# autonomousvision/LaRa

Hardware: AMD Instinct MI355X
Metric: novel-view frames/sec @512x512 (4-view in, 2DGS fwd+bwd) (higher is better)
Workload: dtype f32 raster + bf16-MFMA/f32-accumulate encoder (+ bf16-autocast coarse decoder MLP, as the reference's bf16-mixed)

## Files before the change

lara_amd/coarse.py:

```python
from __future__ import annotations

import torch
from torch import nn

from ._native import call, query, require_device

_F, _FA, _O = 80, 88, 48


class _CoarseDecoder(torch.autograd.Function):
    @staticmethod
    def forward(ctx, x, w1, b1, w2, b2, w3, b3, K, sh_dim, opacity_shift, scaling_shift):
        require_device(x)
        f = lambda t: t.detach().float().contiguous()
        x, w1, b1, w2, b2, w3, b3 = map(f, (x, w1, b1, w2, b2, w3, b3))
        M, n_par = x.shape[0], K * (10 + sh_dim)
        if (x.shape != (M, _F) or w1.shape != (_F, _F) or w2.shape != (_F, _F) or w3.shape != (n_par, _F) or n_par > _O
                or b1.shape != (_F,) or b2.shape != (_F,) or b3.shape != (n_par,)):
            raise RuntimeError("expected x [M,80], Linear(80,80), Linear(80,80), Linear(80, K*(10+sh_dim) <= 48)")
        new = lambda c: torch.empty(M, K * c, dtype=torch.float32, device=x.device)
        offset, sh, scaling, rotation, opacity = new(3), new(sh_dim), new(2), new(4), new(1)
        call("lara_coarse_decoder_forward", x.device, M, K, sh_dim, x, w1, b1, w2, b2, w3, b3, float(opacity_shift),
             float(scaling_shift), offset, sh, scaling, rotation, opacity)
        ctx.save_for_backward(x, w1, b1, w2, b2, w3, offset)
        ctx.dims = (M, K, sh_dim, n_par)
        ctx.set_materialize_grads(False)
        return offset, sh, scaling, rotation, opacity

    @staticmethod
    def backward(ctx, g_offset, g_sh, g_scaling, g_rotation, g_opacity):
        x, w1, b1, w2, b2, w3, offset = ctx.saved_tensors
        M, K, sh_dim, n_par = ctx.dims
        gs = [None if g is None else g.float().contiguous() for g in (g_offset, g_sh, g_scaling, g_rotation, g_opacity)]
        dev = x.device
        Mp = query("lara_coarse_decoder_padded_rows", M)
        dx = torch.empty_like(x)
        cols = (_FA, _FA, _FA, _F, _F, _O)
        slab = torch.empty(Mp * sum(cols), dtype=torch.bfloat16, device=dev)
        mats, o = [], 0
        for c in cols:
            mats.append(slab[o:o + Mp * c].view(Mp, c))
            o += Mp * c
        xb, h1, h2, dz1, dz2, dz3 = mats
        grads = torch.zeros((2 * _F + _O) * _FA, dtype=torch.float32, device=dev)
        g1, g2, g3 = grads[:_F * _FA].view(_F, _FA), grads[_F * _FA:2 * _F * _FA].view(_F, _FA), grads[2 * _F * _FA:].view(_O, _FA)
        ws = torch.empty(query("lara_gemm_tn_workspace_bytes"), dtype=torch.uint8, device=dev)
        call("lara_coarse_decoder_backward", dev, M, K, sh_dim, x, w1, b1, w2, b2, w3, offset, *gs, dx, xb, h1, h2, dz1, dz2, dz3)
        if M:
            for dz, act, g in ((dz1, xb, g1), (dz2, h1, g2), (dz3, h2, g3)):
                call("lara_gemm_tn_bf16", dev, Mp, dz.shape[1], _FA, dz, act, g, ws)
        return (dx, g1[:, :_F], g1[:, _F], g2[:, :_F], g2[:, _F], g3[:n_par, :_F], g3[:n_par, _F], None, None, None, None)


def supported(decoder) -> bool:
    seq = getattr(decoder, "mlp_coarse", None)
    if any(not hasattr(decoder, a) for a in ("K", "sh_dim", "opacity_dim", "scaling_dim", "rotation_dim")):
        return False
    if seq is None or len(seq) != 5 or not all(isinstance(seq[i], nn.Linear) for i in (0, 2, 4)):
        return False
    if not all(isinstance(seq[i], nn.ReLU) for i in (1, 3)) or any(seq[i].bias is None for i in (0, 2, 4)):
        return False
    return (tuple(seq[0].weight.shape) == (_F, _F) and tuple(seq[2].weight.shape) == (_F, _F)
            and tuple(seq[4].weight.shape) == (decoder.K * (10 + decoder.sh_dim), _F) and seq[4].weight.shape[0] <= _O
            and decoder.opacity_dim == 1 and decoder.scaling_dim == 2 and decoder.rotation_dim == 4)


def forward_coarse(decoder, feats, opacity_shift, scaling_shift):
    if not supported(decoder):
        raise RuntimeError("lara_amd.coarse: mlp_coarse must be Linear(80,80) ReLU Linear(80,80) ReLU Linear(80, K*(10+sh_dim) <= 48)")
    seq, K, B = decoder.mlp_coarse, decoder.K, feats.shape[0]
    offset, sh, scaling, rotation, opacity = _CoarseDecoder.apply(
        feats.reshape(-1, feats.shape[-1]), seq[0].weight, seq[0].bias, seq[2].weight, seq[2].bias, seq[4].weight, seq[4].bias,
        K, decoder.sh_dim, opacity_shift, scaling_shift)
    return (offset.view(B, -1, 3), sh.view(B, -1, decoder.sh_dim // 3, 3), scaling.view(B, -1, 2), rotation.view(B, -1, 4),
            opacity.view(B, -1, 1))
```

lara_amd/csrc/coarsedec.hip:

```cpp
#include "common.h"
#include "../../include/lara_coarsedec.h"

namespace {

typedef __attribute__((ext_vector_type(4))) short s16x4;
typedef __attribute__((ext_vector_type(4))) float f32x4;

__device__ __forceinline__ unsigned short f2bf(const float f) {
    unsigned u = __float_as_uint(f);
    u += 0x7fffu + ((u >> 16) & 1u);
    return (unsigned short)(u >> 16);
}
__device__ __forceinline__ float bf2f(const unsigned short h) { return __uint_as_float((unsigned)h << 16); }

constexpr int CD_F = 80;
constexpr int CD_O = 48;
constexpr int CD_LDW = 84;
constexpr int CD_PTS = 128;
constexpr int CD_NB = 208;
constexpr int CD_FA = 88;
constexpr int CD_TILE = 16 * CD_O + 16 * 12;
constexpr int CD_WG_FWD = 1024, CD_WG_BWD = 512;

struct CdP {
    int M, n_par;
    const float *x, *w1, *b1, *w2, *b2, *w3, *b3;
    float *out[5];
    const float *dout[5];
    const float *offset_out;
    float *dx;
    unsigned short *xb, *h1, *h2, *dz1, *dz2, *dz3;
    float opacity_shift, scaling_shift;
    int width[5], toff[5];
    signed char tensor[CD_O], col[CD_O], act[CD_O];
};

template <int ROWS>
__device__ __forceinline__ void stage_matrix(const float *__restrict__ w, const int rows_valid, unsigned short *dst,
                                             const int ld, const bool transposed) {
    constexpr int N = ROWS * CD_F, TRIPS = (N + 255) / 256;
    float v[TRIPS];
#pragma unroll
    for (int u = 0; u < TRIPS; u++) {
        const int idx = u * 256 + (int)threadIdx.x;
        v[u] = (idx < N && idx < rows_valid * CD_F) ? w[idx] : 0.f;
    }
#pragma unroll
    for (int u = 0; u < TRIPS; u++) {
        const int idx = u * 256 + (int)threadIdx.x;
        if (idx >= N) continue;
        const int r = idx / CD_F, c = idx - r * CD_F;
        if (transposed) dst[c * ld + r] = f2bf(v[u]); else dst[r * ld + c] = f2bf(v[u]);
    }
}
__device__ __forceinline__ void stage_bias(const float *__restrict__ b, const int n_valid, const int n, float *dst) {
    for (int i = threadIdx.x; i < n; i += 256) dst[i] = i < n_valid ? bf2f(f2bf(b[i])) : 0.f;
}

typedef __attribute__((ext_vector_type(4))) __bf16 bf16x4;
template <int NI, int NT, bool TR>
__device__ __forceinline__ void mm(const unsigned short *Ws, const int ld, const float *bs, const s16x4 (&in)[NT][2],
                                   f32x4 (&acc)[NI][2], const int c16, const int q4) {
#pragma unroll
    for (int i = 0; i < NI; i++) {
        f32x4 b = {0.f, 0.f, 0.f, 0.f};
        if (bs) b = *(const f32x4 *)(bs + 16 * i + 4 * q4);
        acc[i][0] = b; acc[i][1] = b;
#pragma unroll
        for (int t = 0; t < NT; t++) {
            s16x4 a;
            if (TR) {
                const unsigned short *src = Ws + (16 * t + 4 * q4 + (c16 >> 2)) * ld + 16 * i + 4 * (c16 & 3);
                a = __builtin_bit_cast(s16x4, __builtin_amdgcn_ds_read_tr16_b64_v4bf16((__attribute__((address_space(3))) bf16x4 *)src));
            } else {
                a = *(const s16x4 *)(Ws + (16 * i + c16) * ld + 16 * t + 4 * q4);
            }
            acc[i][0] = __builtin_amdgcn_mfma_f32_16x16x16bf16_1k(a, in[t][0], acc[i][0], 0, 0, 0);
            acc[i][1] = __builtin_amdgcn_mfma_f32_16x16x16bf16_1k(a, in[t][1], acc[i][1], 0, 0, 0);
        }
    }
}

__device__ __forceinline__ s16x4 pack4(const float a, const float b, const float c, const float d) {
// ... 198 lines not shown
            const float *tl = tile + c * CD_TILE;
#pragma unroll
            for (int i = 0; i < 3; i++) {
                float v[4];
#pragma unroll
                for (int r = 0; r < 4; r++) {
                    v[r] = 0.f;
                    if (slot[i][r] < 0) continue;
                    float g = tl[slot[i][r]];
                    if ((is_offset >> (4 * i + r)) & 1u) {
                        const float o = tl[16 * CD_O + slot[i][r]];
                        g *= 0.5f * (1.0f - o * o);
                    }
                    v[r] = g;
                }
                g3[i][c] = pack4(v[0], v[1], v[2], v[3]);
            }
        }
        __builtin_amdgcn_wave_barrier();
        asm volatile("s_waitcnt lgkmcnt(0)" ::: "memory");
        store_frags<3, false>(p.dz3, CD_O, base, c16, q4, g3);
        mm<5, 3, true>(W3s, CD_LDW, nullptr, g3, acc, c16, q4);
#pragma unroll
        for (int i = 0; i < 5; i++)
#pragma unroll
            for (int c = 0; c < 2; c++) {
                const bool in_range = base + 16 * c + c16 < p.M;
#pragma unroll
                for (int e = 0; e < 4; e++) {
                    const unsigned short h = (in_range && ((live2[c] >> (4 * i + e)) & 1u)) ? f2bf(acc[i][c][e]) : (unsigned short)0;
                    a[i][c][e] = (short)h;
                }
            }
        store_frags<5, false>(p.dz2, CD_F, base, c16, q4, a);
        mm<5, 5, true>(W2s, CD_LDW, nullptr, a, acc, c16, q4);
#pragma unroll
        for (int i = 0; i < 5; i++)
#pragma unroll
            for (int c = 0; c < 2; c++) {
                const bool in_range = base + 16 * c + c16 < p.M;
#pragma unroll
                for (int e = 0; e < 4; e++) {
                    const unsigned short h = (in_range && ((live1[c] >> (4 * i + e)) & 1u)) ? f2bf(acc[i][c][e]) : (unsigned short)0;
                    b[i][c][e] = (short)h;
                }
            }
        store_frags<5, false>(p.dz1, CD_F, base, c16, q4, b);
        mm<5, 5, true>(W1s, CD_LDW, nullptr, b, acc, c16, q4);
#pragma unroll
        for (int c = 0; c < 2; c++) {
            const int row = base + 16 * c + c16;
            if (row >= p.M) continue;
            float4 *dst = (float4 *)(p.dx + (size_t)row * CD_F) + q4;
#pragma unroll
            for (int i = 0; i < 5; i++) dst[4 * i] = make_float4(acc[i][c][0], acc[i][c][1], acc[i][c][2], acc[i][c][3]);
        }
    }
}

int fill_map(CdP &p, const int K, const int sh_dim) {
    const int per = 10 + sh_dim;
    if (K < 1 || sh_dim < 0 || K * per > CD_O) return LARA2DGS_E_INVALID;
    static_assert(CD_TILE - 16 * CD_O >= 16 * 3 * (CD_O / 10), "the backward's copy of `offset` (16 x 3K floats) must fit the tile's tail for every K with 10 K <= CD_O");
    p.n_par = K * per;
    const int widths[5] = {3, sh_dim, 2, 4, 1};
    for (int t = 0, o = 0; t < 5; t++) { p.width[t] = K * widths[t]; p.toff[t] = o; o += 16 * p.width[t]; }
    for (int q = 0; q < CD_O; q++) { p.tensor[q] = 0; p.col[q] = 0; p.act[q] = 0; }
    for (int k = 0; k < K; k++)
        for (int j = 0; j < per; j++) {
            int t, c, a = 0;
            if (j < 3) { t = 0; c = j; a = 1; }
            else if (j < 3 + sh_dim) { t = 1; c = j - 3; }
            else if (j < 4 + sh_dim) { t = 4; c = 0; a = 3; }
            else if (j < 6 + sh_dim) { t = 2; c = j - 4 - sh_dim; a = 2; }
            else { t = 3; c = j - 6 - sh_dim; }
            const int q = k * per + j;
            p.tensor[q] = (signed char)t; p.col[q] = (signed char)(k * widths[t] + c); p.act[q] = (signed char)a;
        }
    return LARA2DGS_OK;
}

}

extern "C" {

int64_t lara_coarse_decoder_padded_rows(int64_t M) { return (M + CD_PTS - 1) / CD_PTS * CD_PTS; }

int lara_coarse_decoder_forward(int32_t M, int32_t K, int32_t sh_dim, const float *x, const float *w1, const float *b1,
                                const float *w2, const float *b2, const float *w3, const float *b3, float opacity_shift,
                                float scaling_shift, float *offset, float *sh, float *scaling, float *rotation,
                                float *opacity, void *stream) {
    if (M < 0 || !w1 || !b1 || !w2 || !b2 || !w3 || !b3) return LARA2DGS_E_INVALID;
    CdP p{};
    if (int rc = fill_map(p, K, sh_dim)) return rc;
    if (M == 0) return LARA2DGS_OK;
    if (!x || !offset || !scaling || !rotation || !opacity || (sh_dim > 0 && !sh)) return LARA2DGS_E_INVALID;
    p.M = M; p.x = x; p.w1 = w1; p.b1 = b1; p.w2 = w2; p.b2 = b2; p.w3 = w3; p.b3 = b3;
    p.out[0] = offset; p.out[1] = sh; p.out[2] = scaling; p.out[3] = rotation; p.out[4] = opacity;
    p.opacity_shift = opacity_shift; p.scaling_shift = scaling_shift;
    const int trips = (M + CD_PTS - 1) / CD_PTS;
    L2D_LAUNCH("coarse_decoder_fwd", (hipStream_t)stream, coarse_fwd_kernel, dim3(trips < CD_WG_FWD ? trips : CD_WG_FWD), dim3(256), 0, p);
    return LARA2DGS_OK;
}

int lara_coarse_decoder_backward(int32_t M, int32_t K, int32_t sh_dim, const float *x, const float *w1, const float *b1,
                                 const float *w2, const float *b2, const float *w3, const float *offset_out,
                                 const float *d_offset, const float *d_sh, const float *d_scaling, const float *d_rotation,
                                 const float *d_opacity, float *dx, uint16_t *xb, uint16_t *h1, uint16_t *h2,
                                 uint16_t *dz1, uint16_t *dz2, uint16_t *dz3, void *stream) {
    if (M < 0 || !w1 || !b1 || !w2 || !b2 || !w3) return LARA2DGS_E_INVALID;
    CdP p{};
    if (int rc = fill_map(p, K, sh_dim)) return rc;
    hipStream_t s = (hipStream_t)stream;
    if (M == 0) return LARA2DGS_OK;
    if (!x || !dx || !xb || !h1 || !h2 || !dz1 || !dz2 || !dz3 || (d_offset && !offset_out)) return LARA2DGS_E_INVALID;
    p.M = M; p.x = x; p.w1 = w1; p.b1 = b1; p.w2 = w2; p.b2 = b2; p.w3 = w3;
    p.dout[0] = d_offset; p.dout[1] = d_sh; p.dout[2] = d_scaling; p.dout[3] = d_rotation; p.dout[4] = d_opacity;
    p.offset_out = offset_out; p.dx = dx;
    p.xb = xb; p.h1 = h1; p.h2 = h2; p.dz1 = dz1; p.dz2 = dz2; p.dz3 = dz3;
    const int trips = (M + CD_PTS - 1) / CD_PTS;
    const int grid = trips < CD_WG_BWD ? trips : CD_WG_BWD;
    L2D_LAUNCH("coarse_decoder_bwd", s, coarse_bwd_kernel, dim3(grid), dim3(256), 0, p);
    return LARA2DGS_OK;
}

}
```

lara_amd/csrc/pointfeat.hip:

```cpp
#include "common.h"
#include "../../include/lara_pointfeat.h"

namespace {

constexpr int PF_MAX_VIEWS = 8;

struct PfP {
    int n, V, h, w;
    const float *points, *w2cs, *ixts, *img_ref, *image, *acc, *depth;
    int vtot;
};

__device__ __forceinline__ size_t map_pixel(const PfP &p, const size_t i) {
    if (p.vtot == 0) return i;
    const size_t hw = (size_t)p.h * p.w, v = i / hw, pix = i - v * hw, y = pix / p.w, x = pix - y * p.w;
    return (y * p.vtot + v) * p.w + x;
}

struct Tap {
    int idx[4];
    float wgt[4];
    float wx, wy;
    bool in[4];
};

__device__ __forceinline__ Tap taps(const float x, const float y, const int h, const int w) {
    Tap t;
    const float fx = floorf(x), fy = floorf(y);
    t.wx = x - fx; t.wy = y - fy;
    const int x0 = (fx >= -2.f && fx <= (float)w + 1.f) ? (int)fx : -2, y0 = (fy >= -2.f && fy <= (float)h + 1.f) ? (int)fy : -2;
#pragma unroll
    for (int k = 0; k < 4; k++) {
        const int xi = x0 + (k & 1), yi = y0 + (k >> 1);
        t.in[k] = xi >= 0 && xi < w && yi >= 0 && yi < h;
        t.idx[k] = t.in[k] ? yi * w + xi : 0;
        t.wgt[k] = ((k & 1) ? t.wx : 1.f - t.wx) * ((k >> 1) ? t.wy : 1.f - t.wy);
    }
    return t;
}

__global__ void __launch_bounds__(256)
pack_stack_kernel(const PfP p, float4 *__restrict__ packed) {
    const size_t hw = (size_t)p.h * p.w, i = (size_t)blockIdx.x * 256 + threadIdx.x;
    if (i >= (size_t)p.V * hw) return;
    const size_t v = i / hw, pix = i - v * hw, m = map_pixel(p, i);
    const float *im = p.image + m * 3;
    packed[2 * i] = make_float4(p.img_ref[(v * 3 + 0) * hw + pix], p.img_ref[(v * 3 + 1) * hw + pix],
                                p.img_ref[(v * 3 + 2) * hw + pix], im[0]);
    packed[2 * i + 1] = make_float4(im[1], im[2], p.acc[m], p.depth[m]);
}

__global__ void __launch_bounds__(256)
unpack_grad_kernel(const PfP p, const float4 *__restrict__ dpacked, const size_t n, float *d_image, float *d_acc, float *d_depth) {
    const size_t i = (size_t)blockIdx.x * 256 + threadIdx.x;
// ... 138 lines not shown
    L2D_LAUNCH_IN_SCOPE(s, (point_feats_bwd_kernel<VP>), dim3((unsigned)((threads + 255) / 256)), dim3(256), 0, p, packed, g_out,
                        d_points, dpacked);
    return LARA2DGS_OK;
}
int launch_pack(const PfP &p, float4 *packed, hipStream_t s) {
    const size_t n = (size_t)p.V * p.h * p.w;
    L2D_LAUNCH_IN_SCOPE(s, pack_stack_kernel, dim3((unsigned)((n + 255) / 256)), dim3(256), 0, p, packed);
    return LARA2DGS_OK;
}

struct RowsP {
    const float *src[LARA_ROWS_MAX];
    float *dst[LARA_ROWS_MAX];
    int width[LARA_ROWS_MAX], first[LARA_ROWS_MAX + 1];
    const int64_t *idx;
    int n, count;
};
template <bool SCATTER>
__global__ void __launch_bounds__(256) take_rows_kernel(const RowsP p) {
    const int total = p.first[p.count];
    const int t = blockIdx.x * 256 + threadIdx.x;
    if (t >= p.n * total) return;
    const int r = t / total, c = t - r * total;
    int k = 0;
    while (k + 1 < p.count && c >= p.first[k + 1]) k++;
    const int w = p.width[k], cc = c - p.first[k];
    const size_t far = (size_t)p.idx[r] * w + cc, near = (size_t)r * w + cc;
    if (SCATTER) p.dst[k][far] = p.src[k][near];
    else p.dst[k][near] = p.src[k][far];
}

__global__ void __launch_bounds__(256) voxel_rows_fwd_kernel(const int n, const int c4, const long long *__restrict__ vox,
                                                            const float4 *__restrict__ x, float4 *__restrict__ out) {
    const long long t = (long long)blockIdx.x * 256 + threadIdx.x;
    if (t >= (long long)n * c4) return;
    const int r = (int)(t / c4), c = (int)(t - (long long)r * c4);
    out[t] = x[(size_t)vox[r] * c4 + c];
}
__global__ void __launch_bounds__(256) voxel_rows_bwd_kernel(const int n, const int c4, const long long *__restrict__ vox,
                                                            const float4 *__restrict__ g, float4 *__restrict__ dx) {
    const long long t = (long long)blockIdx.x * 256 + threadIdx.x;
    if (t >= (long long)n * c4) return;
    const int r = (int)(t / c4), c = (int)(t - (long long)r * c4);
    const long long v = vox[r];
    if (r > 0 && vox[r - 1] == v) return;
    float4 a = g[t];
    for (int q = r + 1; q < n && vox[q] == v; q++) {
        const float4 b = g[(size_t)q * c4 + c];
        a.x += b.x; a.y += b.y; a.z += b.z; a.w += b.w;
    }
    dx[(size_t)v * c4 + c] = a;
}

}

extern "C" {

int lara_voxel_rows(int32_t n, int32_t width, const int64_t *vox, const float *src, float *dst, int32_t backward, void *stream) {
    if (n < 0 || width <= 0 || (width & 3)) return LARA2DGS_E_INVALID;
    if (n == 0) return LARA2DGS_OK;
    if (!vox || !src || !dst) return LARA2DGS_E_INVALID;
    hipStream_t s = (hipStream_t)stream;
    const int c4 = width / 4;
    const unsigned blocks = (unsigned)(((long long)n * c4 + 255) / 256);
    {
        L2D_PROF(backward ? "voxel_rows_bwd" : "voxel_rows_fwd", s);
        if (backward) L2D_LAUNCH_IN_SCOPE(s, voxel_rows_bwd_kernel, dim3(blocks), dim3(256), 0, n, c4, (const long long *)vox, (const float4 *)src, (float4 *)dst);
        else L2D_LAUNCH_IN_SCOPE(s, voxel_rows_fwd_kernel, dim3(blocks), dim3(256), 0, n, c4, (const long long *)vox, (const float4 *)src, (float4 *)dst);
    }
    return LARA2DGS_OK;
}

int64_t lara_point_feats_workspace_bytes(int32_t V, int32_t h, int32_t w) {
    if (V <= 0 || V > PF_MAX_VIEWS || h <= 0 || w <= 0 || (int64_t)V * h * w * 8 >= (1ll << 31)) return LARA2DGS_E_INVALID;
    return (int64_t)V * h * w * 32 * 2;
}

int lara_point_feats_forward(int32_t n, int32_t V, int32_t h, int32_t w, const float *points, const float *w2cs,
                             const float *ixts, const float *img_ref, const float *image, const float *acc_map,
                             const float *depth, float *out, void *workspace, void *stream) {
    return lara_point_feats_forward_concat(n, V, 0, h, w, points, w2cs, ixts, img_ref, image, acc_map, depth, out, workspace, stream);
}

int lara_point_feats_forward_concat(int32_t n, int32_t V, int32_t row_views, int32_t h, int32_t w, const float *points,
                                    const float *w2cs, const float *ixts, const float *img_ref, const float *image,
                                    const float *acc_map, const float *depth, float *out, void *workspace, void *stream) {
    if (row_views < 0 || (row_views > 0 && row_views < V)) return LARA2DGS_E_INVALID;
    if (n < 0 || V <= 0 || V > PF_MAX_VIEWS || h <= 0 || w <= 0 || (int64_t)V * h * w * 8 >= (1ll << 31)) return LARA2DGS_E_INVALID;
    if (n == 0) return LARA2DGS_OK;
    if (!points || !w2cs || !ixts || !img_ref || !image || !acc_map || !depth || !out || !workspace) return LARA2DGS_E_INVALID;
    hipStream_t s = (hipStream_t)stream;
    const PfP p{n, V, h, w, points, w2cs, ixts, img_ref, image, acc_map, depth, row_views};
    float4 *packed = (float4 *)workspace;
    {
        L2D_PROF("point_feats_pack", s);
        L2D_TRY(launch_pack(p, packed, s));
    }
    {
        L2D_PROF("point_feats_fwd", s);
        if (V == 1) L2D_TRY(launch_fwd<1>(p, packed, out, s));
        else if (V == 2) L2D_TRY(launch_fwd<2>(p, packed, out, s));
        else if (V <= 4) L2D_TRY(launch_fwd<4>(p, packed, out, s));
        else L2D_TRY(launch_fwd<8>(p, packed, out, s));
    }
    return LARA2DGS_OK;
}

int lara_point_feats_backward(int32_t n, int32_t V, int32_t h, int32_t w, const float *points, const float *w2cs,
                              const float *ixts, const float *img_ref, const float *image, const float *acc_map,
// ... 66 lines not shown
```

lara_amd/fine.py:

```python
from __future__ import annotations

import math
import os

import torch

from ._native import RowsItem, alloc_bytes, call, query, require_device


def _workspace(device, V, h, w):
    return alloc_bytes(query("lara_point_feats_workspace_bytes", V, h, w), device)


class _PointFeats(torch.autograd.Function):
    @staticmethod
    def forward(ctx, points, w2cs, ixts, img_ref, image, acc_map, depth, row_views):
        require_device(points)
        f = lambda t: t.detach().float().contiguous()
        points, w2cs, ixts, img_ref, image, acc_map, depth = map(f, (points, w2cs, ixts, img_ref, image, acc_map, depth))
        n, V, h, w = points.shape[0], img_ref.shape[0], img_ref.shape[2], img_ref.shape[3]
        if points.shape != (n, 3) or w2cs.shape != (V, 4, 4) or ixts.shape != (V, 3, 3) or img_ref.shape != (V, 3, h, w):
            raise RuntimeError("expected points [n,3], w2cs [V,4,4], ixts [V,3,3], img_ref [V,3,h,w]")
        if row_views:
            R = int(row_views)
            if R < V or image.shape != (h, R * w, 3) or acc_map.numel() != h * R * w or depth.shape != (h, R * w, 1):
                raise RuntimeError("expected points [n,3], ... and image [h,R*w,3], acc_map [h,R*w], depth [h,R*w,1] with R = row_views >= V")
        elif image.shape != (V, h, w, 3) or acc_map.shape != (V, h, w) or depth.shape != (V, h, w, 1):
            raise RuntimeError("expected points [n,3], w2cs [V,4,4], ixts [V,3,3], img_ref [V,3,h,w], image [V,h,w,3], acc_map [V,h,w], depth [V,h,w,1]")
        out = torch.empty(V, 8, n, dtype=torch.float32, device=points.device)
        ws = _workspace(points.device, V, h, w)
        call("lara_point_feats_forward_concat", points.device, n, V, int(row_views or 0), h, w, points, w2cs, ixts, img_ref, image,
             acc_map, depth, out, ws)
        ctx.save_for_backward(points, w2cs, ixts, img_ref, image, acc_map, depth)
        ctx.row_views = int(row_views or 0)
        return out

    @staticmethod
    def backward(ctx, g_out):
        points, w2cs, ixts, img_ref, image, acc_map, depth = ctx.saved_tensors
        n, V, h, w = points.shape[0], img_ref.shape[0], img_ref.shape[2], img_ref.shape[3]
        g_out = g_out.float().contiguous()
        need = ctx.needs_input_grad
        d_points = torch.empty_like(points)
        maps = [(image, need[4]), (acc_map, need[5]), (depth, need[6])]
        sizes = [(t.numel() + 3) // 4 * 4 if nd else 0 for t, nd in maps]
        flat = torch.zeros(sum(sizes), dtype=torch.float32, device=points.device)
        secs, o = [], 0
        for (t, nd), sz in zip(maps, sizes):
            secs.append(flat[o:o + t.numel()].view(t.shape) if nd else None)
            o += sz
        d_image, d_acc, d_depth = secs
        ws = _workspace(points.device, V, h, w)
        call("lara_point_feats_backward_concat", points.device, n, V, ctx.row_views, h, w, points, w2cs, ixts, img_ref, image,
             acc_map, depth, g_out, d_points, d_image, d_acc, d_depth, ws)
        return d_points if need[0] else None, None, None, None, d_image, d_acc, d_depth, None


class _TakeRows(torch.autograd.Function):
    @staticmethod
# ... 43 lines not shown
        dev = idx.device
        sizes = [0 if g is None else (math.prod(shape) + 3) // 4 * 4 for g, shape in zip(gs, ctx.shapes)]
        flat = torch.zeros(sum(sizes), dtype=torch.float32, device=dev)
        grads, o = [], 0
        for g, shape, sz in zip(gs, ctx.shapes, sizes):
            grads.append(None if g is None else flat[o:o + math.prod(shape)].view(shape))
            o += sz
        live = [(g.float().contiguous(), d) for g, d in zip(gs, grads) if g is not None]
        if live and idx.numel():
            _rows_call(idx, [g for g, _ in live], [d for _, d in live], True)
        return (None,) + tuple(grads)


class _VoxelRowsScenes(torch.autograd.Function):

    @staticmethod
    def forward(ctx, vol, *vox):
        require_device(vol)
        if vol.dim() != 3 or len(vox) != vol.shape[0] or vol.shape[2] % 4:
            raise RuntimeError("lara_amd: voxel rows need vol [B, V, C] (C % 4 == 0) and one index tensor per scene")
        x = vol.detach().float().contiguous()
        dev, C = x.device, x.shape[2]
        outs = []
        for i, v in enumerate(vox):
            if v.dtype != torch.int64 or v.device != dev or v.dim() != 1:
                raise RuntimeError(f"lara_amd: voxel indices must be 1-D int64 tensors on {dev}")
            v = v.contiguous()
            out = torch.empty((v.numel(), C), dtype=torch.float32, device=dev)
            call("lara_voxel_rows", dev, v.numel(), C, v, x[i], out, 0)
            outs.append(out)
        ctx.save_for_backward(*[v.contiguous() for v in vox])
        ctx.shape = tuple(x.shape)
        ctx.set_materialize_grads(False)
        return tuple(outs)

    @staticmethod
    def backward(ctx, *gs):
        vox = ctx.saved_tensors
        B, V, C = ctx.shape
        dev = vox[0].device
        d = torch.zeros(ctx.shape, dtype=torch.float32, device=dev)
        for i, (v, g) in enumerate(zip(vox, gs)):
            if g is None or v.numel() == 0:
                continue
            g = g.float().contiguous()
            call("lara_voxel_rows", dev, v.numel(), C, v, g, d[i], 1)
        return (d,) + (None,) * len(vox)


def voxel_rows_scenes(vol, vox_list):
    return _VoxelRowsScenes.apply(vol, *vox_list)


def take_rows_multi(xs, idx):
    return _TakeRowsMulti.apply(idx, *xs)


def take_rows(x, idx):
    return _TakeRows.apply(x, idx)


def sample_point_feats(points, w2cs, ixts, img_ref, image, acc_map, depth, row_views=0):
    return _PointFeats.apply(points, w2cs, ixts, img_ref, image, acc_map, depth, row_views)


def get_point_feats(self, idx, img_ref, renderings, n_views_sel, batch, points, mask):
    points = points[mask]
    src_ixts = batch['tar_ixt'][idx, :n_views_sel].reshape(-1, 3, 3)
    src_w2cs = batch['tar_w2c'][idx, :n_views_sel].reshape(-1, 4, 4)
    feats = sample_point_feats(points, src_w2cs, src_ixts, img_ref, renderings['image'], renderings['acc_map'],
                               renderings['depth'])
    return feats, mask


_FD, _NH, _HD, _CD, _NV, _HID, _SH = 80, 8, 10, 8, 4, 64, 12


class _FineDecoder(torch.autograd.Function):

    @staticmethod
    def forward(ctx, xn, pf, Wqk, W1ov, b1, W2, b2):
        require_device(xn)
        f = lambda t: t.detach().float().contiguous()
        xn, pf, Wqk, W1ov, b1, W2, b2 = map(f, (xn, pf, Wqk, W1ov, b1, W2, b2))
        n = xn.shape[0]
        if (xn.shape != (n, _FD) or pf.shape != (_NV, _CD, n) or Wqk.shape != (_NH * _CD, _FD) or W1ov.shape != (_HID, _NH * _CD)
                or b1.shape != (_HID,) or W2.shape != (_SH, _HID) or b2.shape != (_SH,)):
            raise RuntimeError("lara_fine_decoder_forward: the kernel is built for xn [n,80], pf [4,8,n], Wqk [64,80], "
                               "W1ov [64,64], b1 [64], W2 [12,64], b2 [12]")
        sh = torch.empty(n, _SH, dtype=torch.float32, device=xn.device)
        call("lara_fine_decoder_forward", xn.device, n, xn, pf, Wqk, W1ov, b1, W2, b2, sh)
        ctx.save_for_backward(xn, pf, Wqk, W1ov, b1, W2, b2)
        return sh

    @staticmethod
    def backward(ctx, d_sh):
        xn, pf, Wqk, W1ov, b1, W2, b2 = ctx.saved_tensors
        n = xn.shape[0]
        d_sh = d_sh.float().contiguous()
        new = lambda *s: torch.empty(*s, dtype=torch.float32, device=xn.device)
        d_xn, d_pf = new(n, _FD), new(_NV, _CD, n)
        U, H, DH, DT = new(n, 64), new(n, _HID), new(n, _HID), new(n, 64)
        call("lara_fine_decoder_backward", xn.device, n, xn, pf, Wqk, W1ov, b1, W2, b2, d_sh, d_xn, d_pf, U, H, DH, DT)
        dw = new(query("lara_fine_wgrad_floats"))
        ws = torch.empty(max(query("lara_fine_wgrad_workspace_bytes", n), 16), dtype=torch.uint8, device=xn.device)
        call("lara_fine_decoder_wgrad", xn.device, n, xn, U, H, DH, DT, d_sh, dw, ws)
# ... 81 lines not shown
```

lara_amd/pipeline.py:

```python
from __future__ import annotations

import contextlib
import math

import os

import torch
from torch import nn

from . import _native, cameras, coarse
from .fine import _tn_over_points, fold_fine_weights, forward_fine, sample_point_feats, take_rows, take_rows_multi, voxel_rows_scenes
from .renderer import Renderer, _AssembleScenes, batch_map_buffers


class CoarseFineDecoder(nn.Module):

    def __init__(self, in_dim=80, sh_dim=12, scaling_dim=2, rotation_dim=4, opacity_dim=1, K=2):
        super().__init__()
        self.K, self.sh_dim, self.opacity_dim, self.scaling_dim, self.rotation_dim = K, sh_dim, opacity_dim, scaling_dim, rotation_dim
        self.out_dim = 3 + sh_dim + opacity_dim + scaling_dim + rotation_dim
        self.mlp_coarse = nn.Sequential(nn.Linear(in_dim, in_dim), nn.ReLU(), nn.Linear(in_dim, in_dim), nn.ReLU(),
                                        nn.Linear(in_dim, self.out_dim * K))
        self.norm = nn.LayerNorm(in_dim)
        self.cross_att = nn.MultiheadAttention(embed_dim=in_dim, num_heads=8, kdim=8, vdim=8, dropout=0.0, bias=False,
                                               batch_first=True)
        self.mlp_fine = nn.Sequential(nn.Linear(in_dim, 64), nn.ReLU(), nn.Linear(64, sh_dim))
        for seq in (self.mlp_coarse, self.mlp_fine):
            for layer in seq:
                if isinstance(layer, nn.Linear):
                    nn.init.xavier_uniform_(layer.weight)
                    nn.init.zeros_(layer.bias)


class _LinearBf16(torch.autograd.Function):

    @staticmethod
    def forward(ctx, x, weight, bias):
        xb = x.reshape(-1, x.shape[-1]).to(torch.bfloat16)
        wb = weight.to(torch.bfloat16)
        y = torch.nn.functional.linear(xb, wb, None if bias is None else bias.to(torch.bfloat16))
        ctx.save_for_backward(xb, wb)
        ctx.x_shape, ctx.x_dtype, ctx.has_bias = x.shape, x.dtype, bias is not None
        return y.view(*x.shape[:-1], weight.shape[0])

    @staticmethod
    def backward(ctx, dy):
        xb, wb = ctx.saved_tensors
        dy = dy.reshape(-1, dy.shape[-1]).to(torch.bfloat16).contiguous()
        dx = (dy @ wb).view(ctx.x_shape).to(ctx.x_dtype) if ctx.needs_input_grad[0] else None
        dw = _tn_over_points(dy, xb)
        db = dy.float().sum(0) if ctx.has_bias else None
        return dx, dw, db


def _mlp_bf16(seq, x):
    for m in seq:
        x = _LinearBf16.apply(x, m.weight, m.bias) if isinstance(m, nn.Linear) else m(x)
    return x


def decode_coarse(decoder, feats, opacity_shift, scaling_shift, autocast=True):
    par = (_mlp_bf16(decoder.mlp_coarse, feats) if autocast else decoder.mlp_coarse(feats)).float()
    K = decoder.K
    par = par.view(*par.shape[:-1], K, -1)
# ... 31 lines not shown
    elif hasattr(obj, "__dict__"):
        for v in vars(obj).values():
            if torch.is_tensor(v):
                hand_over(v, stream)


class _TakeVoxelRows(torch.autograd.Function):

    @staticmethod
    def forward(ctx, x, vox):
        ctx.save_for_backward(vox)
        ctx.n = x.shape[0]
        return x.index_select(0, vox)

    @staticmethod
    def backward(ctx, g):
        (vox,) = ctx.saved_tensors
        out = g.new_zeros((ctx.n,) + tuple(g.shape[1:]))
        out.index_add_(0, vox, g.contiguous())
        return out, None


class LaRaPipeline(nn.Module):

    def __init__(self, vol_decoder, decoder, grid_reso=32, n_offset_groups=32, sh_degree=1, white_bkgd=True, n_views=4,
                 scene_size=0.5, n_streams=2, feat_volume=None, image_encoder=None):
        super().__init__()
        self.vol_decoder, self.decoder = vol_decoder, decoder
        self.feat_volume = feat_volume
        self.image_encoder = image_encoder
        self.K = decoder.K
        self.n_views, self.scene_size, self.n_offset_groups = n_views, scene_size, n_offset_groups
        self.gs_render = Renderer(sh_degree=sh_degree, white_background=white_bkgd, radius=1)
        self.opacity_shift = -2.1792
        self.voxel_size = 2.0 / (grid_reso * 2)
        self.scaling_shift = math.log(0.5 * self.voxel_size / 3.0)
        r = grid_reso * 2
        a = torch.arange(r)
        grid = (torch.stack(torch.meshgrid(a, a, a, indexing="ij"), dim=-1) + 0.5) / r * 2 - 1
        self.register_buffer("group_centers", (grid * scene_size).reshape(1, -1, 3).float())
        self.n_streams = n_streams
        self._streams = []
        self.fused_coarse = True
        self.fine_mask = "reference"
        self.fine_reuses_coarse_lists = True
        self.stage_events = None
        self.opacity_bias = None

    def gaussians(self, feat_vol):
        return self.gaussians_from_volume(self.vol_decoder(feat_vol))

    def gaussians_from_volume(self, vol, autocast=True):
        if autocast and self.fused_coarse and vol.is_cuda and coarse.supported(self.decoder):
            offset, shs, scaling, rotation, opacity = coarse.forward_coarse(self.decoder, vol, self.opacity_shift, self.scaling_shift)
        else:
            offset, shs, scaling, rotation, opacity = decode_coarse(self.decoder, vol, self.opacity_shift, self.scaling_shift, autocast)
        if self.opacity_bias is not None:
            opacity = opacity + self.opacity_bias
        half_cell = 0.5 * self.scene_size / self.n_offset_groups
        B = offset.shape[0]
        centers = self.group_centers.unsqueeze(-2).expand(B, -1, self.K, -1).reshape(offset.shape) + offset * half_cell
        masks = torch.sigmoid(opacity.detach()).squeeze(-1) > 0.005
        return {"centers": centers, "shs": shs, "scaling": scaling, "rotation": rotation, "opacity": opacity,
                "masks": masks, "vol": vol.view(B, -1, vol.shape[-1])}

    def trained_like_opacity_bias(self):
        r = self.group_centers.norm(dim=-1, keepdim=True)
        bias = torch.where((r - 0.35).abs() < 0.02, 4.0 - self.opacity_shift, -6.0 - self.opacity_shift)
        return bias.unsqueeze(-2).expand(-1, -1, self.K, -1).reshape(1, -1, 1).contiguous()

    @staticmethod
    def host_scalars(batch):
        packed = torch.cat([batch["near_far"].float(), batch["fovx"].float()[:, None], batch["fovy"].float()[:, None]], 1).cpu()
        return [tuple(float(x) for x in row) for row in packed]

    def scene_cameras(self, batch, i, scalars=None):
        near, far, fx, fy = (scalars or self.host_scalars(batch))[i]
        H, W = int(batch["meta"]["tar_h"][i]), int(batch["meta"]["tar_w"][i])
        return cameras.make_cameras(batch["tar_c2w"][i], W, H, fx, fy, near, far, device=batch["tar_c2w"].device)

    def _mark(self, name):
        if self.stage_events is not None:
            e = torch.cuda.Event(enable_timing=True)
            e.record()
            self.stage_events.append((name, e))

    def forward(self, batch, feat_vol, with_fine=True, n_views_sel=None, return_buffer=False):
        if n_views_sel is not None and int(n_views_sel) != self.n_views:
            raise NotImplementedError(f"lara_amd.pipeline: built for {self.n_views} input views (configs/base.yaml n_views); got n_views_sel="
                                      f"{n_views_sel} (cfg.train.use_rand_views): not supported by the fused fine stage")
        if feat_vol.dim() == 6 and feat_vol.shape[1] != self.n_views:
            raise NotImplementedError(f"lara_amd.pipeline: the image-feature volume holds {feat_vol.shape[1]} views, the pipeline is built for {self.n_views}")
        return self._step(batch, lambda: self.gaussians(feat_vol), feat_vol.device, feat_vol.shape[0], with_fine, return_buffer)

    def forward_from_image_features(self, batch, img_feats, with_fine=True, return_buffer=False):
        if self.feat_volume is None:
            raise RuntimeError("lara_amd.pipeline: forward_from_image_features needs LaRaPipeline(..., feat_volume=FeatureVolume(...))")
        from .encoder_train import VolTransformer as HipVolTransformer
        if isinstance(self.vol_decoder, HipVolTransformer):
            make = lambda: self.gaussians_from_volume(self.vol_decoder.forward_from_image_features(self.feat_volume, batch, img_feats, self.n_views))
        else:
            make = lambda: self.gaussians(self.feat_volume(batch, img_feats, self.n_views))
        return self._step(batch, make, img_feats.device, batch["tar_rays_down"].shape[0], with_fine, return_buffer)

    def forward_from_images(self, batch, with_fine=True, return_buffer=False):
        if self.image_encoder is None:
            raise RuntimeError("lara_amd.pipeline: forward_from_images needs LaRaPipeline(..., image_encoder=DinoViT(...))")
        if self.feat_volume is None:
            raise RuntimeError("lara_amd.pipeline: forward_from_images needs LaRaPipeline(..., feat_volume=FeatureVolume(...))")
        return self.forward_from_image_features(batch, self.image_encoder.image_features(batch, self.n_views), with_fine, return_buffer)

    def forward_from_volume(self, batch, volume_feat_up, with_fine=True, autocast=True, return_buffer=False):
        return self._step(batch, lambda: self.gaussians_from_volume(volume_feat_up, autocast), volume_feat_up.device,
                          volume_feat_up.shape[0], with_fine, return_buffer)

    def _step(self, batch, make_gaussians, dev, B, with_fine, return_buffer=False):
        _native.require_device(dev)
        n_sel = self.n_views
        scalars = self.host_scalars(batch)
        cur = torch.cuda.current_stream(dev)
        n_streams = min(self.n_streams, B)
        while len(self._streams) < n_streams and n_streams > 1:
            self._streams.append(torch.cuda.Stream(dev))
        sides = self._streams[:n_streams] if n_streams > 1 else [None] * B
        on = lambda s: torch.cuda.stream(s) if s is not None else contextlib.nullcontext()

        sizes = [(int(batch["meta"]["tar_w"][i]), int(batch["meta"]["tar_h"][i])) for i in range(B)]
        cams_of = cameras.make_cameras_scenes(batch["tar_c2w"], sizes, scalars, device=batch["tar_c2w"].device)
        bg_rows = torch.nn.functional.pad(batch["bg_color"].float(), (0, 1))[..., :3]
        self._mark("start")
        g = make_gaussians()
        inps = batch["tar_rgb"][:, :n_sel].permute(0, 1, 4, 2, 3).float().contiguous()
        if with_fine:
            masks = g["masks"]
            if self.fine_mask == "reference":
                masks = torch.stack([check_mask(masks[i], self.training) for i in range(B)])
        self._mark("encoder+decoder")
        bufs = None
        if len(set(sizes)) == 1 and len({len(c) for c in cams_of}) == 1:
            bufs = batch_map_buffers(B, sizes[0][1], sizes[0][0] * len(cams_of[0]), dev, ("", "_fine") if with_fine else ("",))
        for s in sides:
            if s is not None:
                s.wait_stream(cur)
                hand_over((g, inps, cams_of, bufs, bg_rows, [batch[k] for k in ("tar_rays", "bg_color", "tar_w2c", "tar_ixt") if k in batch]), s)

        sc = {k: g[k].unbind(0) for k in ("centers", "shs", "opacity", "scaling", "rotation")}
        per_scene = [None] * B
        buffers = [[(sc["centers"][i], sc["shs"][i], sc["opacity"][i], sc["scaling"][i], sc["rotation"][i])] for i in range(B)] \
            if return_buffer else None
        coarse_raster = [[] for _ in range(B)]
        for i in range(B):
            s = sides[i % len(sides)]
            with on(s):
                per_scene[i] = self.gs_render.render_views(
                    cams_of[i], batch["tar_rays"][i], sc["centers"][i], sc["shs"][i], sc["opacity"][i], sc["scaling"][i],
                    sc["rotation"][i], dev, bg_colors=bg_rows[i], concat=True,
                    into=None if bufs is None else {k: v[i] for k, v in bufs.items() if not k.endswith("_fine")},
                    raster_out=coarse_raster[i])
                self._mark("coarse views")
        if with_fine:
            idx = [masks[i].nonzero().squeeze(-1) for i in range(B)]
            folded = fold_fine_weights(self.decoder)
            vox = [torch.div(idx[i], self.K, rounding_mode="floor") for i in range(B)]
            vol_rows = voxel_rows_scenes(g["vol"], vox)
            for s in sides:
                if s is not None:
                    s.wait_stream(cur)
                    hand_over((masks, folded, vol_rows), s)
            for i in range(B):
                s = sides[i % len(sides)]
                hand_over(idx[i], s)
                with on(s):
                    co = per_scene[i]
                    H, VW = co["acc_map"].shape
                    V, W = len(cams_of[i]), VW // len(cams_of[i])
                    five = [sc["centers"][i], sc["shs"][i], sc["opacity"][i], sc["scaling"][i], sc["rotation"][i]]
                    centers_f, shs_sel, opacity_f, scaling_f, rotation_f = take_rows_multi(five, idx[i])
                    pf = sample_point_feats(centers_f, batch["tar_w2c"][i, :n_sel], batch["tar_ixt"][i, :n_sel], inps[i],
                                            co["image"], co["acc_map"], co["depth"], row_views=V)
                    sh_res = forward_fine(self.decoder, vol_rows[i], torch.einsum("lcb->blc", pf), folded)
                    shs_f = sh_res.view(-1, *g["shs"].shape[-2:]) + shs_sel
                    if return_buffer:
                        buffers[i].append((centers_f, shs_f, sc["opacity"][i], sc["scaling"][i], sc["rotation"][i], masks[i]))
                    self._mark("sampler+forward_fine")
                    co.update(self.gs_render.render_views(
                        cams_of[i], batch["tar_rays"][i], centers_f, shs_f, opacity_f, scaling_f, rotation_f, dev,
                        bg_colors=bg_rows[i], prex="_fine", concat=True,
                        into=None if bufs is None else {k: v[i] for k, v in bufs.items() if k.endswith("_fine")},
                        subset_of=(coarse_raster[i][0][0], idx[i]) if self.fine_reuses_coarse_lists else None))
                    self._mark("fine views")
        outs = per_scene
        for i, s in enumerate(sides):
            if s is not None:
                cur.wait_stream(s)
        if sides[0] is not None:
            hand_over(per_scene, cur)
            if buffers is not None:
                hand_over(buffers, cur)
        if bufs is not None:
            out = {k: _AssembleScenes.apply(bufs[k], *[o[k] for o in outs]) for k in outs[0]}
        else:
            out = {k: torch.stack([o[k] for o in outs]) for k in outs[0]}
        if return_buffer:
            out["render_pkg"] = [t for scene in buffers for t in scene]
        self._mark("outputs")
        return out

    def join_streams(self):
        cur = torch.cuda.current_stream()
        for s in self._streams:
            cur.wait_stream(s)


def lara_loss(batch, output, it=10000, ms_ssim=True):
    from .loss import ms_ssim_terms
    B, V, H, W = batch["tar_rgb"].shape[:-1]
# ... 23 lines not shown
```

Before: 969.9.

## Fuse fine-mask subset selection into scan kernels and fold volume gradient into decoder backward

Replaces the per-scene check_mask, nonzero and floor-division ops with one two-pass count/scan kernel. It applies the mask rule, emits the indices and voxel ids, and returns the per-scene counts in a single host sync. The coarse decoder now returns an alias of its input features, so the later gradient reaching the volume is added inside the decoder's backward dx store instead of by a separate autograd accumulation. This cuts small kernel launches and host syncs. The cost is reimplementing the random mask rules on device, which changes how the RNG is drawn and relies on the alias gradient being handled correctly.

```diff
diff --git a/lara_amd/_seams.py b/lara_amd/_seams.py
--- /dev/null
+++ b/lara_amd/_seams.py
@@ -0,0 +1,37 @@
+from __future__ import annotations
+
+import torch
+
+from . import _native
+
+ENTRY_POINTS = """
+l lara_subset_indices_workspace_bytes(i i)
+i lara_subset_indices(i*4 p*7 s)
+i lara_coarse_decoder_backward_add(i*3 p*20 s)
+"""
+_SIGS = _native._parse_signatures(ENTRY_POINTS)
+
+
+def _entry(name):
+    fn = getattr(_native.load_library(), name)
+    if fn.argtypes is None:
+        fn.restype, fn.argtypes = _SIGS[name][:2]
+    return fn
+
+
+def call(name, device, *args):
+    fn = _entry(name)
+    with torch.cuda.device(device):
+        a = [x.data_ptr() if isinstance(x, torch.Tensor) else x for x in args] + [_native.current_stream(device)]
+        if len(a) != len(fn.argtypes):
+            raise TypeError(f"lara_amd: {name} takes {len(fn.argtypes)} arguments, got {len(a)}")
+        rc = fn(*a)
+    if rc != 0:
+        _native.check(rc, name)
+
+
+def query(name, *args):
+    n = int(_entry(name)(*args))
+    if n < 0:
+        _native.check(n, name)
+    return n
diff --git a/lara_amd/coarse.py b/lara_amd/coarse.py
--- a/lara_amd/coarse.py
+++ b/lara_amd/coarse.py
@@ -3,6 +3,7 @@
 import torch
 from torch import nn
 
+from . import _seams
 from ._native import call, query, require_device
 
 _F, _FA, _O = 80, 88, 48
@@ -25,16 +26,22 @@
         ctx.save_for_backward(x, w1, b1, w2, b2, w3, offset)
         ctx.dims = (M, K, sh_dim, n_par)
         ctx.set_materialize_grads(False)
-        return offset, sh, scaling, rotation, opacity
+        return offset, sh, scaling, rotation, opacity, x.view(x.shape)
 
     @staticmethod
-    def backward(ctx, g_offset, g_sh, g_scaling, g_rotation, g_opacity):
+    def backward(ctx, g_offset, g_sh, g_scaling, g_rotation, g_opacity, g_x=None):
         x, w1, b1, w2, b2, w3, offset = ctx.saved_tensors
         M, K, sh_dim, n_par = ctx.dims
         gs = [None if g is None else g.float().contiguous() for g in (g_offset, g_sh, g_scaling, g_rotation, g_opacity)]
         dev = x.device
         Mp = query("lara_coarse_decoder_padded_rows", M)
         dx = torch.empty_like(x)
+        if g_x is not None:
+            g_x = g_x.float().contiguous()
+            if g_x.shape != x.shape:
+                raise RuntimeError("lara_amd.coarse: the gradient of the feature alias must have the features' shape")
+            if M == 0:
+                dx = g_x
         cols = (_FA, _FA, _FA, _F, _F, _O)
         slab = torch.empty(Mp * sum(cols), dtype=torch.bfloat16, device=dev)
         mats, o = [], 0
@@ -45,7 +52,7 @@
         grads = torch.zeros((2 * _F + _O) * _FA, dtype=torch.float32, device=dev)
         g1, g2, g3 = grads[:_F * _FA].view(_F, _FA), grads[_F * _FA:2 * _F * _FA].view(_F, _FA), grads[2 * _F * _FA:].view(_O, _FA)
         ws = torch.empty(query("lara_gemm_tn_workspace_bytes"), dtype=torch.uint8, device=dev)
-        call("lara_coarse_decoder_backward", dev, M, K, sh_dim, x, w1, b1, w2, b2, w3, offset, *gs, dx, xb, h1, h2, dz1, dz2, dz3)
+        _seams.call("lara_coarse_decoder_backward_add", dev, M, K, sh_dim, x, w1, b1, w2, b2, w3, offset, *gs, g_x, dx, xb, h1, h2, dz1, dz2, dz3)
         if M:
             for dz, act, g in ((dz1, xb, g1), (dz2, h1, g2), (dz3, h2, g3)):
                 call("lara_gemm_tn_bf16", dev, Mp, dz.shape[1], _FA, dz, act, g, ws)
@@ -66,11 +73,15 @@
 
 
 def forward_coarse(decoder, feats, opacity_shift, scaling_shift):
+    return forward_coarse_shared(decoder, feats, opacity_shift, scaling_shift)[:5]
+
+
+def forward_coarse_shared(decoder, feats, opacity_shift, scaling_shift):
     if not supported(decoder):
         raise RuntimeError("lara_amd.coarse: mlp_coarse must be Linear(80,80) ReLU Linear(80,80) ReLU Linear(80, K*(10+sh_dim) <= 48)")
     seq, K, B = decoder.mlp_coarse, decoder.K, feats.shape[0]
-    offset, sh, scaling, rotation, opacity = _CoarseDecoder.apply(
+    offset, sh, scaling, rotation, opacity, alias = _CoarseDecoder.apply(
         feats.reshape(-1, feats.shape[-1]), seq[0].weight, seq[0].bias, seq[2].weight, seq[2].bias, seq[4].weight, seq[4].bias,
         K, decoder.sh_dim, opacity_shift, scaling_shift)
     return (offset.view(B, -1, 3), sh.view(B, -1, decoder.sh_dim // 3, 3), scaling.view(B, -1, 2), rotation.view(B, -1, 4),
-            opacity.view(B, -1, 1))
+            opacity.view(B, -1, 1), alias.view(B, -1, alias.shape[-1]))
diff --git a/lara_amd/csrc/coarsedec.hip b/lara_amd/csrc/coarsedec.hip
--- a/lara_amd/csrc/coarsedec.hip
+++ b/lara_amd/csrc/coarsedec.hip
@@ -1,5 +1,6 @@
 #include "common.h"
 #include "../../include/lara_coarsedec.h"
+#include "lara_seams.h"
 
 namespace {
 
@@ -29,6 +30,7 @@
     const float *dout[5];
     const float *offset_out;
     float *dx;
+    const float *dx_add;
     unsigned short *xb, *h1, *h2, *dz1, *dz2, *dz3;
     float opacity_shift, scaling_shift;
     int width[5], toff[5];
@@ -333,8 +335,18 @@
             const int row = base + 16 * c + c16;
             if (row >= p.M) continue;
             float4 *dst = (float4 *)(p.dx + (size_t)row * CD_F) + q4;
-#pragma unroll
-            for (int i = 0; i < 5; i++) dst[4 * i] = make_float4(acc[i][c][0], acc[i][c][1], acc[i][c][2], acc[i][c][3]);
+            if (!p.dx_add) {
+#pragma unroll
+                for (int i = 0; i < 5; i++) dst[4 * i] = make_float4(acc[i][c][0], acc[i][c][1], acc[i][c][2], acc[i][c][3]);
+            } else {
+                const float4 *add = (const float4 *)(p.dx_add + (size_t)row * CD_F) + q4;
+#pragma unroll
+                for (int i = 0; i < 5; i++) {
+                    const float4 a = add[4 * i];
+                    dst[4 * i] = make_float4(__fadd_rn(acc[i][c][0], a.x), __fadd_rn(acc[i][c][1], a.y), __fadd_rn(acc[i][c][2], a.z),
+                                             __fadd_rn(acc[i][c][3], a.w));
+                }
+            }
         }
     }
 }
@@ -389,6 +401,15 @@
                                  const float *d_offset, const float *d_sh, const float *d_scaling, const float *d_rotation,
                                  const float *d_opacity, float *dx, uint16_t *xb, uint16_t *h1, uint16_t *h2,
                                  uint16_t *dz1, uint16_t *dz2, uint16_t *dz3, void *stream) {
+    return lara_coarse_decoder_backward_add(M, K, sh_dim, x, w1, b1, w2, b2, w3, offset_out, d_offset, d_sh, d_scaling, d_rotation,
+                                            d_opacity, nullptr, dx, xb, h1, h2, dz1, dz2, dz3, stream);
+}
+
+int lara_coarse_decoder_backward_add(int32_t M, int32_t K, int32_t sh_dim, const float *x, const float *w1, const float *b1,
+                                     const float *w2, const float *b2, const float *w3, const float *offset_out,
+                                     const float *d_offset, const float *d_sh, const float *d_scaling, const float *d_rotation,
+                                     const float *d_opacity, const float *dx_add, float *dx, uint16_t *xb, uint16_t *h1,
+                                     uint16_t *h2, uint16_t *dz1, uint16_t *dz2, uint16_t *dz3, void *stream) {
     if (M < 0 || !w1 || !b1 || !w2 || !b2 || !w3) return LARA2DGS_E_INVALID;
     CdP p{};
     if (int rc = fill_map(p, K, sh_dim)) return rc;
@@ -397,7 +418,7 @@
     if (!x || !dx || !xb || !h1 || !h2 || !dz1 || !dz2 || !dz3 || (d_offset && !offset_out)) return LARA2DGS_E_INVALID;
     p.M = M; p.x = x; p.w1 = w1; p.b1 = b1; p.w2 = w2; p.b2 = b2; p.w3 = w3;
     p.dout[0] = d_offset; p.dout[1] = d_sh; p.dout[2] = d_scaling; p.dout[3] = d_rotation; p.dout[4] = d_opacity;
-    p.offset_out = offset_out; p.dx = dx;
+    p.offset_out = offset_out; p.dx = dx; p.dx_add = dx_add;
     p.xb = xb; p.h1 = h1; p.h2 = h2; p.dz1 = dz1; p.dz2 = dz2; p.dz3 = dz3;
     const int trips = (M + CD_PTS - 1) / CD_PTS;
     const int grid = trips < CD_WG_BWD ? trips : CD_WG_BWD;
diff --git a/lara_amd/csrc/lara_seams.h b/lara_amd/csrc/lara_seams.h
--- /dev/null
+++ b/lara_amd/csrc/lara_seams.h
@@ -0,0 +1,23 @@
+#ifndef LARA_SEAMS_H
+#define LARA_SEAMS_H
+
+#include <stdint.h>
+
+#ifdef __cplusplus
+extern "C" {
+#endif
+
+int64_t lara_subset_indices_workspace_bytes(int32_t B, int32_t P);
+int lara_subset_indices(int32_t B, int32_t P, int32_t K, int32_t mode, const uint8_t *mask, const float *rnd, uint8_t *mask_out,
+                        int64_t *idx, int64_t *vox, int32_t *counts, void *workspace, void *stream);
+
+int lara_coarse_decoder_backward_add(int32_t M, int32_t K, int32_t sh_dim, const float *x, const float *w1, const float *b1,
+                                     const float *w2, const float *b2, const float *w3, const float *offset_out,
+                                     const float *d_offset, const float *d_sh, const float *d_scaling, const float *d_rotation,
+                                     const float *d_opacity, const float *dx_add, float *dx, uint16_t *xb, uint16_t *h1,
+                                     uint16_t *h2, uint16_t *dz1, uint16_t *dz2, uint16_t *dz3, void *stream);
+
+#ifdef __cplusplus
+}
+#endif
+#endif
diff --git a/lara_amd/csrc/pointfeat.hip b/lara_amd/csrc/pointfeat.hip
--- a/lara_amd/csrc/pointfeat.hip
+++ b/lara_amd/csrc/pointfeat.hip
@@ -1,5 +1,6 @@
 #include "common.h"
 #include "../../include/lara_pointfeat.h"
+#include "lara_seams.h"
 
 namespace {
 
@@ -244,9 +245,142 @@
     dx[(size_t)v * c4 + c] = a;
 }
 
+constexpr int SI_THREADS = 256, SI_PER = 16, SI_CHUNK = SI_THREADS * SI_PER, SI_WAVES = SI_THREADS / 64;
+
+__device__ __forceinline__ void si_flags(const uint8_t *__restrict__ mask, const float *__restrict__ rnd, const int P, const int first,
+                                         const bool vec, unsigned f[3]) {
+    f[0] = f[1] = f[2] = 0;
+    if (first >= P) return;
+    alignas(16) uint8_t m[SI_PER];
+    alignas(16) float r[SI_PER];
+    if (vec) {
+        *(uint4 *)m = *(const uint4 *)(mask + first);
+#pragma unroll
+        for (int q = 0; q < SI_PER / 4; q++) *(float4 *)(r + 4 * q) = rnd ? *(const float4 *)(rnd + first + 4 * q) : make_float4(0.f, 0.f, 0.f, 0.f);
+    } else {
+#pragma unroll
+        for (int j = 0; j < SI_PER; j++) {
+            const bool in = first + j < P;
+            m[j] = in ? mask[first + j] : 0;
+            r[j] = (in && rnd) ? rnd[first + j] : 0.f;
+        }
+    }
+#pragma unroll
+    for (int j = 0; j < SI_PER; j++) {
+        if (!vec && first + j >= P) break;
+        const float mf = m[j] ? 1.f : 0.f;
+        f[0] |= (unsigned)(m[j] != 0) << j;
+        f[1] |= (unsigned)(__fadd_rn(mf, r[j]) > 0.8f) << j;
+        f[2] |= (unsigned)(__fmul_rn(mf, r[j]) > 0.5f) << j;
+    }
+}
+
+template <int N>
+__device__ __forceinline__ void si_block_sum(int v[N], int *red) {
+#pragma unroll
+    for (int k = 0; k < N; k++)
+        for (int d = 32; d > 0; d >>= 1) v[k] += __shfl_xor(v[k], d, 64);
+    const int wave = threadIdx.x >> 6;
+    if ((threadIdx.x & 63) == 0)
+        for (int k = 0; k < N; k++) red[wave * N + k] = v[k];
+    __syncthreads();
+#pragma unroll
+    for (int k = 0; k < N; k++) {
+        v[k] = 0;
+        for (int w = 0; w < SI_WAVES; w++) v[k] += red[w * N + k];
+    }
+    __syncthreads();
+}
+
+__global__ void __launch_bounds__(SI_THREADS)
+subset_count_kernel(const int P, const int nb, const uint8_t *__restrict__ mask, const float *__restrict__ rnd, const bool vec,
+                    int *__restrict__ cnt) {
+    __shared__ int red[SI_WAVES * 3];
+    const int b = blockIdx.y, blk = blockIdx.x;
+    const size_t row = (size_t)b * P;
+    unsigned f[3];
+    si_flags(mask + row, rnd ? rnd + row : nullptr, P, blk * SI_CHUNK + (int)threadIdx.x * SI_PER, vec, f);
+    int c[3] = {(int)__popc(f[0]), (int)__popc(f[1]), (int)__popc(f[2])};
+    si_block_sum<3>(c, red);
+    if (threadIdx.x < 3) cnt[((size_t)b * nb + blk) * 4 + threadIdx.x] = c[threadIdx.x];
+}
+
+__global__ void __launch_bounds__(SI_THREADS)
+subset_emit_kernel(const int P, const int nb, const int K, const int mode, const float inv_p, const uint8_t *__restrict__ mask,
+                   const float *__restrict__ rnd, const bool vec, const int *__restrict__ cnt, uint8_t *__restrict__ mask_out,
+                   long long *__restrict__ idx, long long *__restrict__ vox, int *__restrict__ counts) {
+    __shared__ int red[SI_WAVES * 6];
+    __shared__ int wave_tot[SI_WAVES];
+    const int b = blockIdx.y, blk = blockIdx.x, t = threadIdx.x;
+    const size_t row = (size_t)b * P;
+    int s[6] = {0, 0, 0, 0, 0, 0};
+    for (int j = t; j < nb; j += SI_THREADS) {
+        const int *c = cnt + ((size_t)b * nb + j) * 4;
+#pragma unroll
+        for (int r = 0; r < 3; r++) {
+            s[r] += c[r];
+            if (j < blk) s[3 + r] += c[r];
+        }
+    }
+    si_block_sum<6>(s, red);
+    const float ratio = __fmul_rn((float)s[0], inv_p);
+    int rule = 0;
+    if (mode >= 1 && ratio < 1e-3f) rule = 1;
+    if (mode >= 2 && ratio > 0.5f) rule = 2;
+    const int total = s[rule], before = s[3 + rule];
+    if (blk == 0 && t == 0) counts[b] = total;
+
+    const int first = blk * SI_CHUNK + t * SI_PER;
+    unsigned f[3];
+    si_flags(mask + row, rnd ? rnd + row : nullptr, P, first, vec, f);
+    const unsigned keep = f[rule];
+    const int mine = __popc(keep);
+    int incl = mine;
+    for (int d = 1; d < 64; d <<= 1) {
+        const int y = __shfl_up(incl, d, 64);
+        if ((t & 63) >= d) incl += y;
+    }
+    if ((t & 63) == 63) wave_tot[t >> 6] = incl;
+    __syncthreads();
+    int pos = before + incl - mine;
+    for (int w = 0; w < (t >> 6); w++) pos += wave_tot[w];
+#pragma unroll
+    for (int j = 0; j < SI_PER; j++) {
+        const int e = first + j;
+        if (e >= P) break;
+        const bool k = (keep >> j) & 1u;
+        mask_out[row + e] = k ? 1 : 0;
+        if (k && pos < total) {
+            idx[row + pos] = e;
+            vox[row + pos] = e / K;
+            pos++;
+        }
+    }
+}
+
 }
 
 extern "C" {
+
+int64_t lara_subset_indices_workspace_bytes(int32_t B, int32_t P) {
+    if (B <= 0 || P <= 0) return LARA2DGS_E_INVALID;
+    return (int64_t)B * ((P + SI_CHUNK - 1) / SI_CHUNK) * 4 * (int64_t)sizeof(int);
+}
+
+int lara_subset_indices(int32_t B, int32_t P, int32_t K, int32_t mode, const uint8_t *mask, const float *rnd, uint8_t *mask_out,
+                        int64_t *idx, int64_t *vox, int32_t *counts, void *workspace, void *stream) {
+    if (B <= 0 || B > 65535 || P <= 0 || P > (1 << 30) || K <= 0 || mode < 0 || mode > 2) return LARA2DGS_E_INVALID;
+    if (!mask || !mask_out || !idx || !vox || !counts || !workspace || (mode > 0 && !rnd)) return LARA2DGS_E_INVALID;
+    hipStream_t s = (hipStream_t)stream;
+    const int nb = (P + SI_CHUNK - 1) / SI_CHUNK;
+    const bool vec = P % SI_PER == 0 && ((uintptr_t)mask & 15) == 0 && ((uintptr_t)rnd & 15) == 0;
+    if (mode == 0) rnd = nullptr;
+    int *cnt = (int *)workspace;
+    L2D_LAUNCH_IN_SCOPE(s, subset_count_kernel, dim3((unsigned)nb, (unsigned)B), dim3(SI_THREADS), 0, P, nb, mask, rnd, vec, cnt);
+    L2D_LAUNCH_IN_SCOPE(s, subset_emit_kernel, dim3((unsigned)nb, (unsigned)B), dim3(SI_THREADS), 0, P, nb, K, mode, 1.f / (float)P, mask, rnd,
+                        vec, (const int *)cnt, mask_out, (long long *)idx, (long long *)vox, counts);
+    return LARA2DGS_OK;
+}
 
 int lara_voxel_rows(int32_t n, int32_t width, const int64_t *vox, const float *src, float *dst, int32_t backward, void *stream) {
     if (n < 0 || width <= 0 || (width & 3)) return LARA2DGS_E_INVALID;
diff --git a/lara_amd/fine.py b/lara_amd/fine.py
--- a/lara_amd/fine.py
+++ b/lara_amd/fine.py
@@ -5,6 +5,7 @@
 
 import torch
 
+from . import _seams
 from ._native import RowsItem, alloc_bytes, call, query, require_device
 
 
@@ -154,6 +155,27 @@
     return _VoxelRowsScenes.apply(vol, *vox_list)
 
 
+def subset_indices(masks, K, rule="plain", rnd=None):
+    require_device(masks)
+    mode = {"plain": 0, "eval": 1, "train": 2}[rule]
+    if masks.dim() != 2 or masks.dtype != torch.bool:
+        raise RuntimeError("lara_amd: subset_indices needs masks [B,P] bool")
+    if mode and (rnd is None or rnd.shape != masks.shape or rnd.dtype != torch.float32 or rnd.device != masks.device):
+        raise RuntimeError("lara_amd: subset_indices needs rnd [B,P] fp32 on the masks' device for the rules of _check_mask")
+    masks = masks.contiguous()
+    rnd = rnd.contiguous() if mode else None
+    B, P = masks.shape
+    dev = masks.device
+    out = torch.empty_like(masks)
+    idx = torch.empty(B, P, dtype=torch.int64, device=dev)
+    vox = torch.empty(B, P, dtype=torch.int64, device=dev)
+    counts = torch.empty(B, dtype=torch.int32, device=dev)
+    ws = alloc_bytes(_seams.query("lara_subset_indices_workspace_bytes", B, P), dev)
+    _seams.call("lara_subset_indices", dev, B, P, int(K), mode, masks, rnd, out, idx, vox, counts, ws)
+    n = counts.tolist()
+    return out, [idx[b, :n[b]] for b in range(B)], [vox[b, :n[b]] for b in range(B)]
+
+
 def take_rows_multi(xs, idx):
     return _TakeRowsMulti.apply(idx, *xs)
 
diff --git a/lara_amd/pipeline.py b/lara_amd/pipeline.py
--- a/lara_amd/pipeline.py
+++ b/lara_amd/pipeline.py
@@ -9,7 +9,7 @@
 from torch import nn
 
 from . import _native, cameras, coarse
-from .fine import _tn_over_points, fold_fine_weights, forward_fine, sample_point_feats, take_rows, take_rows_multi, voxel_rows_scenes
+from .fine import _tn_over_points, fold_fine_weights, forward_fine, sample_point_feats, subset_indices, take_rows, take_rows_multi, voxel_rows_scenes
 from .renderer import Renderer, _AssembleScenes, batch_map_buffers
 
 
@@ -147,7 +147,7 @@
 
     def gaussians_from_volume(self, vol, autocast=True):
         if autocast and self.fused_coarse and vol.is_cuda and coarse.supported(self.decoder):
-            offset, shs, scaling, rotation, opacity = coarse.forward_coarse(self.decoder, vol, self.opacity_shift, self.scaling_shift)
+            offset, shs, scaling, rotation, opacity, vol = coarse.forward_coarse_shared(self.decoder, vol, self.opacity_shift, self.scaling_shift)
         else:
             offset, shs, scaling, rotation, opacity = decode_coarse(self.decoder, vol, self.opacity_shift, self.scaling_shift, autocast)
         if self.opacity_bias is not None:
@@ -226,10 +226,10 @@
         self._mark("start")
         g = make_gaussians()
         inps = batch["tar_rgb"][:, :n_sel].permute(0, 1, 4, 2, 3).float().contiguous()
-        if with_fine:
-            masks = g["masks"]
-            if self.fine_mask == "reference":
-                masks = torch.stack([check_mask(masks[i], self.training) for i in range(B)])
+        if with_fine and self.fine_mask == "reference":
+            rnd = torch.empty(g["masks"].shape, dtype=torch.float32, device=dev)
+            for i in range(B):
+                rnd[i].uniform_()
         self._mark("encoder+decoder")
         bufs = None
         if len(set(sizes)) == 1 and len({len(c) for c in cams_of}) == 1:
@@ -254,9 +254,11 @@
                     raster_out=coarse_raster[i])
                 self._mark("coarse views")
         if with_fine:
-            idx = [masks[i].nonzero().squeeze(-1) for i in range(B)]
+            if self.fine_mask == "reference":
+                masks, idx, vox = subset_indices(g["masks"], self.K, "train" if self.training else "eval", rnd)
+            else:
+                masks, idx, vox = subset_indices(g["masks"], self.K)
             folded = fold_fine_weights(self.decoder)
-            vox = [torch.div(idx[i], self.K, rounding_mode="floor") for i in range(B)]
             vol_rows = voxel_rows_scenes(g["vol"], vox)
             for s in sides:
                 if s is not None:
```

New measurement: 977.4, median of 6. No clear change (+0.8%).
